# wenbowen123/iros20-6d-pose-tracking

Measured on AMD Instinct MI355X. Metric: RGB-D pair inferences/sec (176x176), higher is better.
Workload: dtype f32; 1 GPU; configs[1]: batch=64 synthetic 176x176 RGB-D pairs per GPU, random-init Se3TrackNet (reference state_dict surface), stage=full; pairs_per_gpu=64, global_batch=64, stage=full, frames=resident in HBM

## Files before the change

iros20-6d-pose-tracking_amd/csrc/api.cpp:

```cpp
#include <cmath>
#include <thread>
#include <type_traits>
#include <cstdio>
#include <cstdlib>
#include <chrono>
#include <cstring>
#include <map>
#include <mutex>
#include <set>
#include <string>
#include <vector>

#include "hip_buffers.h"
#include "pose_align_plan.h"
#include "pose_errors_plan.h"
#include "pose_grid_plan.h"
#include "pose_search_plan.h"
#include "se3tn_internal.h"
#include "tex_pyramid.h"
#include "track_plan.h"
#include "weights.h"

using namespace se3tn;

// ... 35 lines not shown
  const float* blob = nullptr;
  BlobLayout L;
  DeviceBuf<float> inA, inB;
  DeviceBuf<float> stem;
  DeviceBuf<float> pool, t64, q64;
  DeviceBuf<float> ab, ab_t;
  DeviceBuf<float> head, head_t;
  DeviceBuf<float> head_f;
  unsigned written = 0;
  InferPlan plan;
  DeviceBuf<float> logits;
  DeviceBuf<float> fcpart;
  bool keep_intermediates = false;
  int auto_tile_override[2] = {0, 0};
  int gemmp = -1;
  bool wino_fuse = true;
  DeviceBuf<float> part;
  int tail_parts_ch = 16;
  bool tail_parts = true;
  bool small_kernels = true;
  int wino_min_batch = SE3TN_WINOGRAD_DEFAULT_MIN_BATCH;
  int wino_tile = SE3TN_WINOGRAD_DEFAULT_TILE;
  int wino_tile_derived = 0;
  DeviceBuf<float> wino_u[4];
  DeviceBuf<float> wino_u6[4];
  const float* wino6_blob = nullptr;
  DeviceBuf<float> wino_v, wino_m;
  const float* wino_blob = nullptr;
  int wino64_min_batch = SE3TN_TRUNK_WINOGRAD_DEFAULT_MIN_BATCH;
  int wino64_min_fill = SE3TN_TRUNK_WINOGRAD_DEFAULT_MIN_FILL;
// ... 129 lines not shown
                                 c->wino64_u[i].get() + g * per_g, s.cin, s.cout, 2, st));
  }
  HIPCHK(hipStreamSynchronize(st));
  c->wino64_blob = c->blob;
  return SE3TN_OK;
}

static int wino_prepare(se3tn_ctx* c, hipStream_t st) {
  DeviceGuard dg(c->device);
  HIPCHK(dg.err);
  if (int rc = wino64_prepare(c, st)) return rc;
  if (c->wino_min_batch <= 0 || c->max_batch < c->wino_min_batch) return SE3TN_OK;
  if (!c->wino_v) {
    HIPCHK(c->wino_v.alloc(wino_ws_floats(c->max_batch)));
    HIPCHK(c->wino_m.alloc(wino_ws_floats(c->max_batch)));
    for (int i = 0; i < 4; ++i) {
      const Conv3& s = conv_specs()[kWinoConvs[i]];
      HIPCHK(c->wino_u[i].alloc((size_t)s.groups * 36 * s.cin * s.cout));
    }
  }
  const int tile = c->wino_tile == 2 ? 2 : 4;
  if (c->blob && (c->wino_tile == 6 || c->wino_tile == SE3TN_WINOGRAD_TILE_AUTO || c->wino_tile == SE3TN_WINOGRAD_TILE_6_4) &&
      c->wino6_blob != c->blob) {
    for (int i = 0; i < 4; ++i) {
      const Conv3& s = conv_specs()[kWinoConvs[i]];
      if (!c->wino_u6[i]) HIPCHK(c->wino_u6[i].alloc((size_t)s.groups * 64 * s.cin * s.cout));
      for (int g = 0; g < s.groups; ++g)
        HIPCHK(launch_wino_weights(c->blob + c->L.conv_w[kWinoConvs[i]] + (size_t)g * conv3_words(s.cin, s.cout),
                                   c->wino_u6[i].get() + (size_t)g * 64 * s.cin * s.cout, s.cin, s.cout, 6, st));
    }
// ... 145 lines not shown
const char* se3tn_last_error(void) { return g_err.c_str(); }

int se3tn_create(int device, int max_batch, se3tn_ctx** out) {
  if (!out || max_batch < 1) return fail(SE3TN_E_ARG, "se3tn_create: bad argument");
  if (max_batch > SE3TN_MAX_BATCH_LIMIT)
    return fail(SE3TN_E_ARG, "se3tn_create: max_batch " + std::to_string(max_batch) + " exceeds SE3TN_MAX_BATCH_LIMIT (" +
                                 std::to_string(SE3TN_MAX_BATCH_LIMIT) + "): run larger sets as several calls");
  se3tn_ctx* c = new se3tn_ctx();
  c->device = device;
  c->max_batch = max_batch;
  c->L = blob_layout();
  c->SL = split_layout();
  if (const char* e = std::getenv("SE3TN_WINOGRAD_AUTO_TILE_AB2")) c->auto_tile_override[0] = (std::atoi(e) == 4 || std::atoi(e) == 6) ? std::atoi(e) : 0;
  if (const char* e = std::getenv("SE3TN_WINOGRAD_AUTO_TILE_HEADS")) c->auto_tile_override[1] = (std::atoi(e) == 4 || std::atoi(e) == 6) ? std::atoi(e) : 0;
  if (const char* e = std::getenv("SE3TN_WINO_GEMMP")) c->gemmp = std::atoi(e) != 0 ? 1 : 0;
  if (const char* e = std::getenv("SE3TN_WINOGRAD_FUSE")) c->wino_fuse = std::atoi(e) != 0;
  if (const char* e = std::getenv("SE3TN_TRUNK_WINOGRAD")) c->wino64_min_batch = std::atoi(e);
  if (const char* e = std::getenv("SE3TN_TRUNK_WINOGRAD_FILL")) c->wino64_min_fill = std::atoi(e);
  for (int i = 0; i < 8; ++i) { c->mean[i] = 0.0; c->stdv[i] = 1.0; }
  if (device >= 0) {
    hipDeviceProp_t prop;
    hipError_t e = hipGetDeviceProperties(&prop, device);
    if (e != hipSuccess) { delete c; return hipfail(e, "hipGetDeviceProperties"); }
    if (std::strncmp(prop.gcnArchName, "gfx950", 6) != 0) {
      std::string a = prop.gcnArchName;
      delete c;
      return fail(SE3TN_E_DEVICE, "device is " + a + ", this library is built for gfx950 only");
    }
    if (prop.multiProcessorCount > 0) c->num_cus = prop.multiProcessorCount;
    e = hipSetDevice(device);
// ... 311 lines not shown
    a.per_img = 1;
    std::memcpy(a.img_off, ip->off, sizeof(a.img_off));
  }
}
static void fill_wino_args(se3tn_ctx* c, const ConvRow& r, int tile, int n, const float* W, bool split, WinoArgs& w) {
  const Conv3& s = conv_specs()[r.id];
  const int ws = wino_slot(r.id);
  w = WinoArgs{};
  w.in = tensor_ptr(c, r.in, split); w.bias = W + c->L.conv_b[r.id]; w.res = tensor_ptr(c, r.res, split); w.out = tensor_ptr(c, r.out, split);
  w.U = tile == 6 ? c->wino_u6[ws].get() : c->wino_u[ws].get();
  w.V = c->wino_v.get(); w.Mw = c->wino_m.get();
  w.in_ld = r.in.ld; w.res_ld = r.res.ld; w.out_ld = r.out.ld;
  w.m = tile; w.nf = (tile + 2) * (tile + 2);
  w.H = r.hin; w.W = r.hin; w.th = (r.hin + tile - 1) / tile; w.tw = w.th;
  w.n = n; w.T = n * w.th * w.tw;
  w.C = s.cin; w.Cout = s.cout; w.groups = s.groups;
  w.in_gs = r.in.gs; w.res_gs = r.res.gs; w.out_gs = r.out.gs; w.bias_gs = s.cout;
  w.u_gs = (long long)w.nf * s.cin * s.cout;
  if (split) {
    w.split = 1;
    w.U = c->wino_us[ws].get(); w.uscale = c->wino_usc[ws].get();
    w.overflow = c->overflow.get();
  }
}

static int infer_launch(se3tn_ctx* c, const float* A, const float* B, int n, int layout, float* trans, float* rot,
                        const double* poseA, double* poseB, void* stream);

int se3tn_enable_graphs(se3tn_ctx* c, int on) {
  if (!c || c->device < 0) return fail(SE3TN_E_ARG, "se3tn_enable_graphs: no device context");
// ... 1593 lines not shown
```

iros20-6d-pose-tracking_amd/csrc/se3tn_internal.h:

```cpp
#pragma once
#include <hip/hip_runtime.h>
#include <stddef.h>
#include <stdint.h>

#include "../../include/se3tracknet.h"
#include "infer_plan.h"

namespace se3tn {

struct BlobLayout {
  size_t stem_w;
  size_t stem_b;
  size_t conv_w[NUM_CONV3];
  size_t conv_b[NUM_CONV3];
  size_t fc_w;
  size_t fc_b;
  size_t total;
};

constexpr int HEADER_WORDS = 64;
constexpr uint32_t BLOB_MAGIC = 0x53453354u;
constexpr uint32_t BLOB_VERSION = 7;

struct SplitLayout {
// ... 85 lines not shown
  const float* res;
  float* out;
  float* V;
  float* Mw;
  int in_ld, res_ld, out_ld;
  int H, W;
  int m, nf;
  int th, tw;
  int n, T;
  int C, Cout, groups;
  int in_gs, res_gs, out_gs, bias_gs;
  long long u_gs;
  int split;
  const float* uscale;
  int* overflow;
};

struct TailArgs {
  const float* fc_w;
  const float* fc_b;
  float* logits;
  float* fcpart;
  float* trans;
  float* rot;
  const double* poseA;
  double* poseB;
  double tn, rn;
};

struct CropArgs {
// ... 230 lines not shown
```

iros20-6d-pose-tracking_amd/csrc/wino_mfma.hip:

```cpp
#include "mfma_common.h"
#include "pose_device.h"

#ifndef WINO4_VEC
#define WINO4_VEC 2
#endif
#ifndef WINO_MID_CS_AB
#define WINO_MID_CS_AB 32
#endif
#ifndef WINO_MID_CS_H
#define WINO_MID_CS_H 32
#endif

#ifdef SE3TN_GEMMP_TRACE
__device__ unsigned long long se3tn_gemmp_trace[8 * 64 * 5];
extern "C" int se3tn_debug_gemmp_trace(void* host_out, size_t bytes) {
  return (int)hipMemcpyFromSymbol(host_out, HIP_SYMBOL(se3tn_gemmp_trace), bytes, 0, hipMemcpyDeviceToHost);
}
#define GP_STAMP(K, I) if (blockIdx.x == 0 && lane == 0 && (K) < 64) ::se3tn_gemmp_trace[(wid * 64 + (K)) * 5 + (I)] = __builtin_amdgcn_s_memtime();
#else
#define GP_STAMP(K, I)
#endif
#ifdef SE3TN_WG_TRACE
__device__ unsigned long long se3tn_wg_trace[8 * 4096];
extern "C" int se3tn_debug_wg_trace(void* host_out, size_t bytes, int clear) {
// ... 87 lines not shown
  *reinterpret_cast<hv*>(p_ + 64) = l;
  return bad;
}

struct TileId { int t, cv, n, ty, tx; };
__device__ __forceinline__ TileId tile_of(int idx, int cvn, int th, int tw) {
  TileId r;
  r.cv = idx % cvn; r.t = idx / cvn;
  const int tpi = th * tw;
  r.n = r.t / tpi;
  const int rem = r.t - r.n * tpi;
  r.ty = rem / tw; r.tx = rem - r.ty * tw;
  return r;
}

template <int M, int VEC, int SP = 0>
__global__ __launch_bounds__(256) void wino_input_kernel(const WinoArgs a) {
  constexpr int N = M + 2;
  typedef typename VecT<VEC>::type vec;
  const int cvn = a.C / VEC;
  const int idx = blockIdx.x * 256 + threadIdx.x;
  if (idx >= a.T * cvn) return;
  const int g = blockIdx.y;
  const TileId id = tile_of(idx, cvn, a.th, a.tw);
  const int Hp = a.H + 2, Wp = a.W + 2;
  const float* __restrict__ src = a.in + (size_t)g * a.in_gs + (SP ? 0 : id.cv * VEC);
  float bt[N][N][VEC];
  if constexpr (M == 6) {
    static_assert(SP == 0, "F(6x6) is a float32 path");
#pragma unroll
// ... 37 lines not shown
      __builtin_memcpy(d[r][s], &v, sizeof(v));
    }
#pragma unroll
  for (int i = 0; i < N; ++i)
#pragma unroll
    for (int s = 0; s < N; ++s)
#pragma unroll
      for (int e = 0; e < VEC; ++e) {
        float acc = 0.f;
        bool first = true;
#pragma unroll
        for (int r = 0; r < N; ++r) axpy(acc, wino_bt<M>(i, r), d[r][s][e], first);
        bt[i][s][e] = acc;
      }
  }
  float* __restrict__ dst = a.V + ((size_t)g * a.nf * a.T + id.t) * a.C + (SP ? 0 : id.cv * VEC);
  const size_t fs = (size_t)a.T * a.C;
  bool bad = false;
#pragma unroll
  for (int i = 0; i < N; ++i)
#pragma unroll
    for (int j = 0; j < N; ++j) {
      float o[VEC];
#pragma unroll
      for (int e = 0; e < VEC; ++e) {
        float acc = 0.f;
        bool first = true;
#pragma unroll
        for (int s = 0; s < N; ++s) axpy(acc, wino_bt<M>(j, s), bt[i][s][e], first);
        o[e] = acc;
      }
      if (SP) {
        bad |= store_split_vec<VEC>(dst + (size_t)(N * i + j) * fs, 0, a.C, id.cv * VEC, o);
        continue;
      }
      vec v;
      __builtin_memcpy(&v, o, sizeof(v));
      *reinterpret_cast<vec*>(dst + (size_t)(N * i + j) * fs) = v;
    }
  if (SP && bad) atomicOr(a.overflow, 1);
}

template <int M, int VEC, int EPI, int SP = 0>
__global__ __launch_bounds__(256) void wino_output_kernel(const WinoArgs a) {
  constexpr int N = M + 2;
  typedef typename VecT<VEC>::type vec;
  const int cvn = a.Cout / VEC;
  const int idx = blockIdx.x * 256 + threadIdx.x;
  if (idx >= a.T * cvn) return;
  const int g = blockIdx.y;
  const TileId id = tile_of(idx, cvn, a.th, a.tw);
  const int Hp = a.H + 2, Wp = a.W + 2;
  const float* __restrict__ src = a.Mw + ((size_t)g * a.nf * a.T + id.t) * a.Cout + id.cv * VEC;
  const size_t fs = (size_t)a.T * a.Cout;
  float rr[M][M][VEC];
  if constexpr (EPI == 1 && SP == 0) {
    const float* __restrict__ res0 = a.res + (size_t)g * a.res_gs + id.cv * VEC;
#pragma unroll
    for (int i = 0; i < M; ++i)
#pragma unroll
      for (int j = 0; j < M; ++j) {
        int oy = M * id.ty + i, ox = M * id.tx + j;
        oy = oy < a.H ? oy : a.H - 1; ox = ox < a.W ? ox : a.W - 1;
        const vec v = *reinterpret_cast<const vec*>(res0 + (size_t)((id.n * Hp + oy + 1) * Wp + ox + 1) * a.res_ld);
        __builtin_memcpy(rr[i][j], &v, sizeof(v));
      }
  }
  float u[M][N][VEC];
#pragma unroll
  for (int s = 0; s < N; ++s) {
    float m[N][VEC];
#pragma unroll
    for (int r = 0; r < N; ++r) {
      const vec v = *reinterpret_cast<const vec*>(src + (size_t)(N * r + s) * fs);
      __builtin_memcpy(m[r], &v, sizeof(v));
    }
#pragma unroll
    for (int i = 0; i < M; ++i)
#pragma unroll
      for (int e = 0; e < VEC; ++e) {
        float acc = 0.f;
        bool first = true;
#pragma unroll
        for (int r = 0; r < N; ++r) axpy(acc, wino_at<M>(i, r), m[r][e], first);
        u[i][s][e] = acc;
      }
  }
  float b[VEC];
  {
    const vec v = *reinterpret_cast<const vec*>(a.bias + (size_t)g * a.bias_gs + id.cv * VEC);
    __builtin_memcpy(b, &v, sizeof(v));
  }
  const float* __restrict__ res = (EPI == 1) ? a.res + (size_t)g * a.res_gs + (SP ? 0 : id.cv * VEC) : nullptr;
  float* __restrict__ out = a.out + (size_t)g * a.out_gs + (SP ? 0 : id.cv * VEC);
  bool bad = false;
  if constexpr (SP == 0) __builtin_amdgcn_s_waitcnt(0x0F70);
#pragma unroll
  for (int i = 0; i < M; ++i)
#pragma unroll
    for (int j = 0; j < M; ++j) {
      const int oy = M * id.ty + i, ox = M * id.tx + j;
      if (oy >= a.H || ox >= a.W) continue;
      const size_t pix = (size_t)((id.n * Hp + oy + 1) * Wp + ox + 1);
      float r[VEC];
      if (EPI == 1) {
        if (SP) {
// ... 55 lines not shown
__global__ __launch_bounds__(256, 2) void wino_gemm_kernel(const WinoArgs a) {
  constexpr int BM = WM * PT * 32, BN = WN * CT * 32;
  constexpr int NCH = CIN / 32;
  constexpr int BUF = (BM + BN) * 32;
  static_assert(WM * WN == 4, "4 waves");
  extern __shared__ __attribute__((aligned(16))) float smem[];

  const int tid = threadIdx.x;
  const int lane = tid & 63;
  const int wid = __builtin_amdgcn_readfirstlane(tid >> 6);
  const int wm = wid / WN, wn = wid % WN;
  const int l31 = lane & 31, hh = lane >> 5;

  const int panels = a.Cout / BN, mtiles = (a.T + BM - 1) / BM;
  const int nt = blockIdx.x % panels, rest = blockIdx.x / panels;
  const int mt = rest % mtiles, b = rest / mtiles;
  const int g = b / a.nf, f = b - g * a.nf;
  const int m0 = mt * BM, n0 = nt * BN;
  const float* __restrict__ Vb = a.V + (size_t)b * a.T * CIN;
  const float* __restrict__ Ub = a.U + (size_t)g * a.u_gs + ((size_t)f * a.Cout + n0) * 32;
  const int mlast = a.T - 1;

  const int r0 = tid >> 3;
  const int c4 = (tid & 7) ^ ((r0 >> 1) & 7);
  unsigned pvoff[BM / 32];
#pragma unroll
  for (int j = 0; j < BM / 32; ++j) pvoff[j] = (unsigned)((min(m0 + r0 + 32 * j, mlast) * CIN + c4 * 4) * 4);
  const unsigned wvoff = (unsigned)((r0 * 32 + c4 * 4) * 4);
  const unsigned lds0 = __builtin_amdgcn_readfirstlane(lds_addr_of(smem));

#define ISSUE_TILE(CH, BUFI)                                                                         \
  {                                                                                                  \
    const float* pb_ = Vb + (CH) * 32;                                                               \
    const unsigned lb_ = lds0 + (unsigned)(((BUFI) * BUF + wid * 256) * 4);                          \
    _Pragma("unroll") for (int j_ = 0; j_ < BM / 32; ++j_) glds16<0>(pb_, pvoff[j_], lb_ + j_ * 4096); \
    const float* tb_ = Ub + (size_t)(CH) * a.nf * a.Cout * 32;                                       \
// ... 84 lines not shown
__global__ __launch_bounds__(512, 2) void wino_gemmp_kernel(const WinoArgs a, int total_tiles) {
  constexpr int BM = 128, BN = 256;
  constexpr int WN = 4, PT = 2, CT = 2;
  constexpr int VP = BM / 64;
  constexpr int NCH = CIN / 32;
  constexpr int BUF = (BM + BN) * 32;
  static_assert(NCH % 2 == 0, "the double buffer's parity must be the same at every tile start");
  extern __shared__ __attribute__((aligned(16))) float smem[];

  const int tid = threadIdx.x;
  const int lane = tid & 63;
  const int wid = __builtin_amdgcn_readfirstlane(tid >> 6);
  const int wm = wid / WN, wn = wid % WN;
  const int l31 = lane & 31, hh = lane >> 5;
  const int panels = a.Cout / BN, mtiles = (a.T + BM - 1) / BM, tpp = panels * mtiles;
  const int mlast = a.T - 1;

  const int r0 = tid >> 3;
  const int c4 = (tid & 7) ^ ((r0 >> 1) & 7);
  const unsigned wvoff = (unsigned)((r0 * 32 + c4 * 4) * 4);
  const unsigned lds0 = __builtin_amdgcn_readfirstlane(lds_addr_of(smem));

  auto decode = [&](int v, int& b, int& m0, int& n0) {
    const int xcd = v & 7, s = v >> 3;
    const int q = s / tpp, r = s - q * tpp;
    b = q * 8 + xcd;
    n0 = (r % panels) * BN;
    m0 = (r / panels) * BM;
  };
  const float* Vb;
  const float* Ub;
  unsigned pvoff[VP];
  auto set_tile = [&](int b, int m0, int n0) {
    const int g = b / a.nf, f = b - g * a.nf;
    Vb = a.V + (size_t)b * a.T * CIN;
    Ub = a.U + (size_t)g * a.u_gs + ((size_t)f * a.Cout + n0) * 32;
#pragma unroll
    for (int j = 0; j < VP; ++j) pvoff[j] = (unsigned)((min(m0 + r0 + 64 * j, mlast) * CIN + c4 * 4) * 4);
  };
#define ISSUE_TILEP(CH, BUFI)                                                                        \
  {                                                                                                  \
    const float* pb_ = Vb + (CH) * 32;                                                               \
    const unsigned lb_ = lds0 + (unsigned)(((BUFI) * BUF + wid * 256) * 4);                          \
    _Pragma("unroll") for (int j_ = 0; j_ < VP; ++j_) glds16<0>(pb_, pvoff[j_], lb_ + j_ * 8192);     \
    const float* tb_ = Ub + (size_t)(CH) * a.nf * a.Cout * 32;                                       \
    _Pragma("unroll") for (int j_ = 0; j_ < 4; ++j_) glds16<0>(tb_ + 2048 * j_, wvoff, lb_ + BM * 128 + j_ * 8192); \
  }

  const int X = (l31 >> 1) & 7;
  const int lo = (hh ^ (X & 1)) * 4, xk = X >> 1;
  const int fo0 = ((0 ^ xk) << 3) + lo, fo1 = ((1 ^ xk) << 3) + lo, fo2 = ((2 ^ xk) << 3) + lo, fo3 = ((3 ^ xk) << 3) + lo;

  f32x16 acc[PT][CT];
#pragma unroll
  for (int i = 0; i < PT; ++i)
#pragma unroll
    for (int j = 0; j < CT; ++j)
#pragma unroll
      for (int e = 0; e < 16; ++e) acc[i][j][e] = 0.f;

  int v = blockIdx.x;
  if (v >= total_tiles) return;
  int b, m0, n0;
  decode(v, b, m0, n0);
  set_tile(b, m0, n0);
  ISSUE_TILEP(0, 0)
  wait_dma_and_barrier();

  int kstep_ = 0;
  (void)kstep_;
  while (true) {
    const int vn = v + gridDim.x;
    const bool more = vn < total_tiles;
    const int cb = b, cm0 = m0, cn0 = n0;
#pragma unroll 1
    for (int ch = 0; ch < NCH; ++ch) {
      const int buf = ch & 1;
      GP_STAMP(kstep_, 0)
      if (ch + 1 < NCH) {
        ISSUE_TILEP(ch + 1, buf ^ 1)
      } else if (more) {
        decode(vn, b, m0, n0);
        set_tile(b, m0, n0);
        ISSUE_TILEP(0, buf ^ 1)
      }
      GP_STAMP(kstep_, 1)
      const float* pP = smem + buf * BUF + (wm * PT * 32 + l31) * 32;
      const float* pW = smem + buf * BUF + (BM + wn * CT * 32 + l31) * 32;
#define FOG(G) ((G) == 0 ? fo0 : (G) == 1 ? fo1 : (G) == 2 ? fo2 : fo3)
#define PXF(G) *reinterpret_cast<const float4*>(pP + i * 1024 + FOG(G))
#define WTF(G) *reinterpret_cast<const float4*>(pW + j * 1024 + FOG(G))
      SE3TN_MMA_GROUP(PT, CT, PXF(0), WTF(0))
      SE3TN_MMA_GROUP(PT, CT, PXF(1), WTF(1))
      SE3TN_MMA_GROUP(PT, CT, PXF(2), WTF(2))
      SE3TN_MMA_GROUP(PT, CT, PXF(3), WTF(3))
#undef PXF
#undef WTF
#undef FOG
// ... 3 lines not shown
        GP_STAMP(kstep_, 3)
        __syncthreads();
      }
      GP_STAMP(kstep_, 4)
      ++kstep_;
    }
    float* __restrict__ Mb = a.Mw + (size_t)cb * a.T * a.Cout;
#pragma unroll
    for (int i = 0; i < PT; ++i) {
      const int m = cm0 + (wm * PT + i) * 32 + l31;
#pragma unroll
      for (int j = 0; j < CT; ++j)
#pragma unroll
        for (int q = 0; q < 4; ++q) {
          const int c = cn0 + (wn * CT + j) * 32 + q * 8 + hh * 4;
          if (m <= mlast)
            *reinterpret_cast<float4*>(Mb + (size_t)m * a.Cout + c) =
                make_float4(acc[i][j][4 * q + 0], acc[i][j][4 * q + 1], acc[i][j][4 * q + 2], acc[i][j][4 * q + 3]);
#pragma unroll
          for (int e = 0; e < 4; ++e) acc[i][j][4 * q + e] = 0.f;
        }
    }
    if (!more) break;
    v = vn;
  }
#undef ISSUE_TILEP
}

template <> struct VecT<1> { typedef float type; };

template <int M, int TH, int CS, int VEC, int SP = 0>
__global__ __launch_bounds__(((TH * TH * (CS / VEC) + 63) / 64) * 64) void wino_mid_kernel(const WinoArgs a, float* __restrict__ keep) {
  constexpr int N = M + 2, HP = M * TH + 2, NT = TH * TH, CP = CS / VEC, ITEMS = NT * CP;
  typedef typename VecT<VEC>::type vec;
  static_assert(SP == 0 || (M == 4 && VEC == 2), "the f16x3 blocks are F(4x4) with channel pairs");
  extern __shared__ __attribute__((aligned(16))) float act[];
  const int n = blockIdx.x, c0 = blockIdx.y * CS, g = blockIdx.z;
  const int tid = threadIdx.x;
  for (int i = tid; i < HP * HP * CS / 4; i += blockDim.x) reinterpret_cast<float4*>(act)[i] = make_float4(0.f, 0.f, 0.f, 0.f);
  __syncthreads();
  const int tile = tid / CP, cp = tid - tile * CP;
  const int ty = tile / TH, tx = tile - ty * TH;
  const bool active = tid < ITEMS;
  const int t = n * NT + tile;
  const int Hp = a.H + 2, Wp = a.W + 2;
  if (active) {
    const float* __restrict__ src = a.Mw + ((size_t)g * a.nf * a.T + t) * a.Cout + c0 + cp * VEC;
    const size_t fs = (size_t)a.T * a.Cout;
    float u[M][N][VEC];
#pragma unroll
    for (int s = 0; s < N; ++s) {
      float m[N][VEC];
#pragma unroll
      for (int r = 0; r < N; ++r) {
        const vec v = *reinterpret_cast<const vec*>(src + (size_t)(N * r + s) * fs);
        __builtin_memcpy(m[r], &v, sizeof(v));
      }
#pragma unroll
      for (int i = 0; i < M; ++i)
#pragma unroll
        for (int e = 0; e < VEC; ++e) {
          float acc = 0.f;
          bool first = true;
#pragma unroll
          for (int r = 0; r < N; ++r) axpy(acc, wino_at<M>(i, r), m[r][e], first);
          u[i][s][e] = acc;
        }
    }
    float b[VEC];
    {
      const vec v = *reinterpret_cast<const vec*>(a.bias + (size_t)g * a.bias_gs + c0 + cp * VEC);
      __builtin_memcpy(b, &v, sizeof(v));
    }
    float* __restrict__ kp = keep ? keep + (size_t)g * a.out_gs + c0 + cp * VEC : nullptr;
#pragma unroll
    for (int i = 0; i < M; ++i)
#pragma unroll
      for (int j = 0; j < M; ++j) {
        const int oy = M * ty + i, ox = M * tx + j;
        if (oy >= a.H || ox >= a.W) continue;
        float o[VEC];
#pragma unroll
        for (int e = 0; e < VEC; ++e) {
          float acc = 0.f;
          bool first = true;
#pragma unroll
          for (int s = 0; s < N; ++s) axpy(acc, wino_at<M>(j, s), u[i][s][e], first);
          acc += b[e];
// ... 15 lines not shown
      for (int r = 0; r < N; ++r) {
        const vec v = *reinterpret_cast<const vec*>(act + ((M * ty + r) * HP + M * tx + s) * CS + cp * VEC);
        __builtin_memcpy(d[r], &v, sizeof(v));
      }
#pragma unroll
      for (int i = 0; i < N; ++i)
#pragma unroll
        for (int e = 0; e < VEC; ++e) {
          float acc = 0.f;
          bool first = true;
#pragma unroll
          for (int r = 0; r < N; ++r) axpy(acc, wino_bt<M>(i, r), d[r][e], first);
          bt[i][s][e] = acc;
        }
    }
    float* __restrict__ dst = a.V + ((size_t)g * a.nf * a.T + t) * a.C + (SP ? 0 : c0 + cp * VEC);
    const size_t fs = (size_t)a.T * a.C;
    bool bad = false;
#pragma unroll
    for (int i = 0; i < N; ++i)
#pragma unroll
      for (int j = 0; j < N; ++j) {
        float o[VEC];
#pragma unroll
        for (int e = 0; e < VEC; ++e) {
          float acc = 0.f;
          bool first = true;
#pragma unroll
          for (int s = 0; s < N; ++s) axpy(acc, wino_bt<M>(j, s), bt[i][s][e], first);
          o[e] = acc;
        }
        if constexpr (SP != 0) {
          bad |= store_split_vec<VEC>(dst + (size_t)(N * i + j) * fs, 0, a.C, c0 + cp * VEC, o);
        } else {
          vec v;
          __builtin_memcpy(&v, o, sizeof(v));
          *reinterpret_cast<vec*>(dst + (size_t)(N * i + j) * fs) = v;
        }
      }
    if (SP && bad) atomicOr(a.overflow, 1);
  }
}

__device__ __forceinline__ float wave_sum64(float v) {
#pragma unroll
  for (int o = 32; o > 0; o >>= 1) v += __shfl_xor(v, o, 64);
  return v;
}

template <int M, int TH, int CS, int SP = 0>
__global__ __launch_bounds__(((TH * TH * (CS / 2) + 63) / 64) * 64) void wino_tail_kernel(const WinoArgs a, float* __restrict__ keep,
                                                                                         const float* __restrict__ fc_w,
                                                                                         float* __restrict__ fcpart) {
  constexpr int N = M + 2, NT = TH * TH, CP = CS / 2, ITEMS = NT * CP;
  static_assert(SP == 0 || M == 4, "the f16x3 blocks are F(4x4)");
  static_assert(CP == 32, "the FC partials are reduced inside one half-wave");
  __shared__ float red[NT][CP][2];
  const int n = blockIdx.x, sl = blockIdx.y, g = blockIdx.z, tid = threadIdx.x;
  const int tile = tid / CP, cp = tid - tile * CP;
  const int c = sl * CS + cp * 2;
  const int Hp = a.H + 2, Wp = a.W + 2;
  if (tid < ITEMS) {
    const int ty = tile / TH, tx = tile - ty * TH;
    const size_t fs = (size_t)a.T * a.Cout;
    const float* __restrict__ src = a.Mw + ((size_t)g * a.nf * a.T + n * NT + tile) * a.Cout + c;
    const float* __restrict__ res = a.res + (size_t)g * a.res_gs + (SP ? 0 : c);
    float* __restrict__ kp = keep ? keep + (size_t)g * a.out_gs + c : nullptr;
    const float2 b = *reinterpret_cast<const float2*>(a.bias + (size_t)g * a.bias_gs + c);
    float2 rr[M][M];
    if constexpr (SP == 0) {
#pragma unroll
      for (int i = 0; i < M; ++i)
#pragma unroll
        for (int j = 0; j < M; ++j) {
          int oy = M * ty + i, ox = M * tx + j;
          oy = oy < a.H ? oy : a.H - 1; ox = ox < a.W ? ox : a.W - 1;
          rr[i][j] = *reinterpret_cast<const float2*>(res + (size_t)((n * Hp + oy + 1) * Wp + ox + 1) * a.res_ld);
        }
    }
    float u[M][N][2];
#pragma unroll
    for (int s = 0; s < N; ++s) {
      float m[N][2];
#pragma unroll
      for (int r = 0; r < N; ++r) {
        const float2 v = *reinterpret_cast<const float2*>(src + (size_t)(N * r + s) * fs);
        m[r][0] = v.x; m[r][1] = v.y;
      }
#pragma unroll
      for (int i = 0; i < M; ++i)
#pragma unroll
        for (int e = 0; e < 2; ++e) {
          float acc = 0.f;
          bool first = true;
#pragma unroll
          for (int r = 0; r < N; ++r) axpy(acc, wino_at<M>(i, r), m[r][e], first);
          u[i][s][e] = acc;
        }
    }
    float sum[2] = {0.f, 0.f};
#pragma unroll
    for (int i = 0; i < M; ++i)
#pragma unroll
      for (int j = 0; j < M; ++j) {
        const int oy = M * ty + i, ox = M * tx + j;
        if (oy >= a.H || ox >= a.W) continue;
        const size_t pix = (size_t)((n * Hp + oy + 1) * Wp + ox + 1);
        float2 r;
        if (SP) {
          float rr[2];
          load_split_vec<2>(res, pix, a.res_ld, c, rr);
          r = make_float2(rr[0], rr[1]);
        } else {
// ... 70 lines not shown
}

template <int CIN, int WM, int WN, int PT, int CT, int MM = MM_F32>
static hipError_t launch_gemm(const WinoArgs& a, hipStream_t st) {
  static PerDeviceOnce attr;
  auto kern = wino_gemm_kernel<CIN, WM, WN, PT, CT, MM>;
  constexpr int BM = WM * PT * 32, BN = WN * CT * 32;
  const size_t lds = 2 * (BM + BN) * 32 * sizeof(float);
  bool* done = attr.current();
  if (!done || !*done) {
    hipError_t e = hipFuncSetAttribute(reinterpret_cast<const void*>(kern),
                                       hipFuncAttributeMaxDynamicSharedMemorySize, (int)lds);
    if (e != hipSuccess) return e;
    if (done) *done = true;
  }
  const int grid = (a.Cout / BN) * ((a.T + BM - 1) / BM) * a.groups * a.nf;
  hipLaunchKernelGGL(kern, dim3(grid), dim3(256), lds, st, a);
  return hipGetLastError();
}

template <int CIN>
static hipError_t launch_gemmp(const WinoArgs& a, int total_tiles, int grid, hipStream_t st) {
  static PerDeviceOnce attr;
  auto kern = wino_gemmp_kernel<CIN>;
  const size_t lds = 2 * (128 + 256) * 32 * sizeof(float);
  bool* done = attr.current();
  if (!done || !*done) {
    hipError_t e = hipFuncSetAttribute(reinterpret_cast<const void*>(kern), hipFuncAttributeMaxDynamicSharedMemorySize, (int)lds);
    if (e != hipSuccess) return e;
    if (done) *done = true;
  }
  hipLaunchKernelGGL(kern, dim3(grid), dim3(512), lds, st, a, total_tiles);
  return hipGetLastError();
}

template <int CIN>
static hipError_t launch_gemm_planned(const WinoArgs& a, const GemmPlan& g, hipStream_t st) {
  if (g.kind == GemmPlan::PERSISTENT) {
    if (a.split || a.Cout % 256 != 0 || g.grid < 1 || g.tiles != (a.Cout / 256) * ((a.T + 127) / 128) * a.groups * a.nf) return hipErrorInvalidValue;
    return launch_gemmp<CIN>(a, g.tiles, g.grid, st);
  }
  if (g.kind != GemmPlan::ROWS96 && g.kind != GemmPlan::ROWS128) return hipErrorInvalidValue;
  const bool r96 = g.kind == GemmPlan::ROWS96;
  if (a.split) return r96 ? launch_gemm<CIN, 1, 4, 3, 1, MM_F16X3>(a, st) : launch_gemm<CIN, 2, 2, 2, 2, MM_F16X3>(a, st);
  return r96 ? launch_gemm<CIN, 1, 4, 3, 1>(a, st) : launch_gemm<CIN, 2, 2, 2, 2>(a, st);
}

template <int M, int VEC>
static hipError_t launch_transformed(const WinoArgs& a, const GemmPlan& g, int epi, hipStream_t st) {
  hipLaunchKernelGGL((wino_input_kernel<M, VEC>), dim3((a.T * (a.C / VEC) + 255) / 256, a.groups), dim3(256), 0, st, a);
  hipError_t e = hipGetLastError();
  if (e != hipSuccess) return e;
  e = a.C == 256 ? launch_gemm_planned<256>(a, g, st) : launch_gemm_planned<512>(a, g, st);
  if (e != hipSuccess) return e;
// ... 93 lines not shown
```

Baseline: 41850 pairs/s.

## Skip dead Winograd F(6,3) transform planes for partial boundary tiles

For 6x6-output Winograd tiles, the last row and column of the 8x8 transform only contribute to outputs that are needed when the tile fits fully inside the image. The change reorders V/M rows per plane class (finite, row-infinity, column-infinity), so tiles that do not need those planes are packed out of the GEMM range. The input transform, GEMM (standard and persistent), and output transform then skip the unneeded rows. This is meant to reduce GEMM work and memory traffic on the boundary planes, at the cost of more complex indexing and tile decoding. A debug poison option is also added.

```diff
diff --git a/iros20-6d-pose-tracking_amd/csrc/api.cpp b/iros20-6d-pose-tracking_amd/csrc/api.cpp
--- a/iros20-6d-pose-tracking_amd/csrc/api.cpp
+++ b/iros20-6d-pose-tracking_amd/csrc/api.cpp
@@ -73,6 +73,8 @@
   bool keep_intermediates = false;
   int auto_tile_override[2] = {0, 0};
   int gemmp = -1;
+  bool wino_full_planes = false;
+  bool wino_poison = false;
   bool wino_fuse = true;
   DeviceBuf<float> part;
   int tail_parts_ch = 16;
@@ -232,6 +234,10 @@
   if (!c->wino_v) {
     HIPCHK(c->wino_v.alloc(wino_ws_floats(c->max_batch)));
     HIPCHK(c->wino_m.alloc(wino_ws_floats(c->max_batch)));
+    if (c->wino_poison) {
+      HIPCHK(hipMemset(c->wino_v.get(), 0xFF, c->wino_v.count() * sizeof(float)));
+      HIPCHK(hipMemset(c->wino_m.get(), 0xFF, c->wino_m.count() * sizeof(float)));
+    }
     for (int i = 0; i < 4; ++i) {
       const Conv3& s = conv_specs()[kWinoConvs[i]];
       HIPCHK(c->wino_u[i].alloc((size_t)s.groups * 36 * s.cin * s.cout));
@@ -407,6 +413,8 @@
   if (const char* e = std::getenv("SE3TN_WINOGRAD_AUTO_TILE_AB2")) c->auto_tile_override[0] = (std::atoi(e) == 4 || std::atoi(e) == 6) ? std::atoi(e) : 0;
   if (const char* e = std::getenv("SE3TN_WINOGRAD_AUTO_TILE_HEADS")) c->auto_tile_override[1] = (std::atoi(e) == 4 || std::atoi(e) == 6) ? std::atoi(e) : 0;
   if (const char* e = std::getenv("SE3TN_WINO_GEMMP")) c->gemmp = std::atoi(e) != 0 ? 1 : 0;
+  if (const char* e = std::getenv("SE3TN_WINO_FULL_PLANES")) c->wino_full_planes = std::atoi(e) != 0;
+  if (const char* e = std::getenv("SE3TN_WINO_POISON")) c->wino_poison = std::atoi(e) != 0;
   if (const char* e = std::getenv("SE3TN_WINOGRAD_FUSE")) c->wino_fuse = std::atoi(e) != 0;
   if (const char* e = std::getenv("SE3TN_TRUNK_WINOGRAD")) c->wino64_min_batch = std::atoi(e);
   if (const char* e = std::getenv("SE3TN_TRUNK_WINOGRAD_FILL")) c->wino64_min_fill = std::atoi(e);
@@ -748,6 +756,7 @@
   w.m = tile; w.nf = (tile + 2) * (tile + 2);
   w.H = r.hin; w.W = r.hin; w.th = (r.hin + tile - 1) / tile; w.tw = w.th;
   w.n = n; w.T = n * w.th * w.tw;
+  w.trim = plan_wino_trim(w.H, w.W, tile, w.th, w.tw, n, c->wino_full_planes);
   w.C = s.cin; w.Cout = s.cout; w.groups = s.groups;
   w.in_gs = r.in.gs; w.res_gs = r.res.gs; w.out_gs = r.out.gs; w.bias_gs = s.cout;
   w.u_gs = (long long)w.nf * s.cin * s.cout;
diff --git a/iros20-6d-pose-tracking_amd/csrc/se3tn_internal.h b/iros20-6d-pose-tracking_amd/csrc/se3tn_internal.h
--- a/iros20-6d-pose-tracking_amd/csrc/se3tn_internal.h
+++ b/iros20-6d-pose-tracking_amd/csrc/se3tn_internal.h
@@ -5,6 +5,7 @@
 
 #include "../../include/se3tracknet.h"
 #include "infer_plan.h"
+#include "wino_trim_plan.h"
 
 namespace se3tn {
 
@@ -123,6 +124,7 @@
   int split;
   const float* uscale;
   int* overflow;
+  WinoTrim trim;
 };
 
 struct TailArgs {
diff --git a/iros20-6d-pose-tracking_amd/csrc/wino_mfma.hip b/iros20-6d-pose-tracking_amd/csrc/wino_mfma.hip
--- a/iros20-6d-pose-tracking_amd/csrc/wino_mfma.hip
+++ b/iros20-6d-pose-tracking_amd/csrc/wino_mfma.hip
@@ -125,6 +125,92 @@
   return r;
 }
 
+struct TileRows { int ra, rc; bool need_r, need_c; };
+template <int M>
+__device__ __forceinline__ TileRows tile_rows(const WinoArgs& a, int t, int img, int ty, int tx) {
+  TileRows r{t, t, true, true};
+  if constexpr (M == 6) {
+    r.ra = wino_trim_row(a.trim, WINO_PLANES_FINITE, a.n, a.th, a.tw, img, ty, tx);
+    r.rc = wino_trim_row(a.trim, WINO_PLANES_COL_INF, a.n, a.th, a.tw, img, ty, tx);
+    r.need_r = ty < a.trim.ny;
+    r.need_c = tx < a.trim.nx;
+  }
+  return r;
+}
+
+template <int VEC>
+__device__ __forceinline__ void out_rows6(const float* __restrict__ src_a, const float* __restrict__ src_c, size_t fs, const TileRows& tr,
+                                          float (&u)[6][8][VEC]) {
+  typedef typename VecT<VEC>::type vec;
+  float mr[8][VEC], mc[7][VEC];
+  if (tr.need_r) {
+#pragma unroll
+    for (int s = 0; s < 8; ++s) {
+      const vec v = *reinterpret_cast<const vec*>(src_a + (size_t)(56 + s) * fs);
+      __builtin_memcpy(mr[s], &v, sizeof(v));
+    }
+  }
+  if (tr.need_c) {
+#pragma unroll
+    for (int r = 0; r < 7; ++r) {
+      const vec v = *reinterpret_cast<const vec*>(src_c + (size_t)(8 * r + 7) * fs);
+      __builtin_memcpy(mc[r], &v, sizeof(v));
+    }
+  }
+  float m[7][7][VEC];
+  const float* __restrict__ p = src_a;
+#pragma unroll
+  for (int r = 0; r < 7; ++r) {
+#pragma unroll
+    for (int s = 0; s < 7; ++s) {
+      const vec v = *reinterpret_cast<const vec*>(p);
+      __builtin_memcpy(m[r][s], &v, sizeof(v));
+      p += fs;
+    }
+    p += fs;
+  }
+  __builtin_amdgcn_sched_barrier(0);
+#pragma unroll
+  for (int s = 0; s < 7; ++s)
+#pragma unroll
+    for (int i = 0; i < 6; ++i)
+#pragma unroll
+      for (int e = 0; e < VEC; ++e) {
+        float acc = 0.f;
+        bool first = true;
+#pragma unroll
+        for (int r = 0; r < 7; ++r) axpy(acc, wino_at<6>(i, r), m[r][s][e], first);
+        u[i][s][e] = acc;
+      }
+#pragma unroll
+  for (int i = 0; i < 6; ++i)
+#pragma unroll
+    for (int e = 0; e < VEC; ++e) u[i][7][e] = 0.f;
+  if (tr.need_c) {
+#pragma unroll
+    for (int i = 0; i < 6; ++i)
+#pragma unroll
+      for (int e = 0; e < VEC; ++e) {
+        float acc = 0.f;
+        bool first = true;
+#pragma unroll
+        for (int r = 0; r < 7; ++r) axpy(acc, wino_at<6>(i, r), mc[r][e], first);
+        u[i][7][e] = acc;
+      }
+  }
+  if (tr.need_r) {
+#pragma unroll
+    for (int s = 0; s < 8; ++s)
+#pragma unroll
+      for (int i = 0; i < 6; ++i)
+#pragma unroll
+        for (int e = 0; e < VEC; ++e) {
+          bool first = false;
+          axpy(u[i][s][e], wino_at<6>(i, 7), mr[s][e], first);
+        }
+  }
+}
+
 template <int M, int VEC, int SP = 0>
 __global__ __launch_bounds__(256) void wino_input_kernel(const WinoArgs a) {
   constexpr int N = M + 2;
@@ -192,13 +278,18 @@
         bt[i][s][e] = acc;
       }
   }
-  float* __restrict__ dst = a.V + ((size_t)g * a.nf * a.T + id.t) * a.C + (SP ? 0 : id.cv * VEC);
+  const TileRows tr = tile_rows<M>(a, id.t, id.n, id.ty, id.tx);
+  float* __restrict__ dst = a.V + ((size_t)g * a.nf * a.T + tr.ra) * a.C + (SP ? 0 : id.cv * VEC);
+  float* __restrict__ dst_c = a.V + ((size_t)g * a.nf * a.T + tr.rc) * a.C + (SP ? 0 : id.cv * VEC);
   const size_t fs = (size_t)a.T * a.C;
   bool bad = false;
 #pragma unroll
   for (int i = 0; i < N; ++i)
 #pragma unroll
     for (int j = 0; j < N; ++j) {
+      if constexpr (M == 6) {
+        if (i == N - 1 ? !tr.need_r : (j == N - 1 && !tr.need_c)) continue;
+      }
       float o[VEC];
 #pragma unroll
       for (int e = 0; e < VEC; ++e) {
@@ -208,13 +299,14 @@
         for (int s = 0; s < N; ++s) axpy(acc, wino_bt<M>(j, s), bt[i][s][e], first);
         o[e] = acc;
       }
+      float* __restrict__ d = (M == 6 && j == N - 1 && i < N - 1 ? dst_c : dst) + (size_t)(N * i + j) * fs;
       if (SP) {
-        bad |= store_split_vec<VEC>(dst + (size_t)(N * i + j) * fs, 0, a.C, id.cv * VEC, o);
+        bad |= store_split_vec<VEC>(d, 0, a.C, id.cv * VEC, o);
         continue;
       }
       vec v;
       __builtin_memcpy(&v, o, sizeof(v));
-      *reinterpret_cast<vec*>(dst + (size_t)(N * i + j) * fs) = v;
+      *reinterpret_cast<vec*>(d) = v;
     }
   if (SP && bad) atomicOr(a.overflow, 1);
 }
@@ -229,7 +321,8 @@
   const int g = blockIdx.y;
   const TileId id = tile_of(idx, cvn, a.th, a.tw);
   const int Hp = a.H + 2, Wp = a.W + 2;
-  const float* __restrict__ src = a.Mw + ((size_t)g * a.nf * a.T + id.t) * a.Cout + id.cv * VEC;
+  const TileRows tr = tile_rows<M>(a, id.t, id.n, id.ty, id.tx);
+  const float* __restrict__ src = a.Mw + ((size_t)g * a.nf * a.T + tr.ra) * a.Cout + id.cv * VEC;
   const size_t fs = (size_t)a.T * a.Cout;
   float rr[M][M][VEC];
   if constexpr (EPI == 1 && SP == 0) {
@@ -244,30 +337,34 @@
         __builtin_memcpy(rr[i][j], &v, sizeof(v));
       }
   }
-  float u[M][N][VEC];
-#pragma unroll
-  for (int s = 0; s < N; ++s) {
-    float m[N][VEC];
-#pragma unroll
-    for (int r = 0; r < N; ++r) {
-      const vec v = *reinterpret_cast<const vec*>(src + (size_t)(N * r + s) * fs);
-      __builtin_memcpy(m[r], &v, sizeof(v));
-    }
-#pragma unroll
-    for (int i = 0; i < M; ++i)
-#pragma unroll
-      for (int e = 0; e < VEC; ++e) {
-        float acc = 0.f;
-        bool first = true;
-#pragma unroll
-        for (int r = 0; r < N; ++r) axpy(acc, wino_at<M>(i, r), m[r][e], first);
-        u[i][s][e] = acc;
-      }
-  }
   float b[VEC];
   {
     const vec v = *reinterpret_cast<const vec*>(a.bias + (size_t)g * a.bias_gs + id.cv * VEC);
     __builtin_memcpy(b, &v, sizeof(v));
+  }
+  float u[M][N][VEC];
+  if constexpr (M == 6) {
+    out_rows6<VEC>(src, a.Mw + ((size_t)g * a.nf * a.T + tr.rc) * a.Cout + id.cv * VEC, fs, tr, u);
+  } else {
+#pragma unroll
+  for (int s = 0; s < N; ++s) {
+    float m[N][VEC];
+#pragma unroll
+    for (int r = 0; r < N; ++r) {
+      const vec v = *reinterpret_cast<const vec*>(src + (size_t)(N * r + s) * fs);
+      __builtin_memcpy(m[r], &v, sizeof(v));
+    }
+#pragma unroll
+    for (int i = 0; i < M; ++i)
+#pragma unroll
+      for (int e = 0; e < VEC; ++e) {
+        float acc = 0.f;
+        bool first = true;
+#pragma unroll
+        for (int r = 0; r < N; ++r) axpy(acc, wino_at<M>(i, r), m[r][e], first);
+        u[i][s][e] = acc;
+      }
+  }
   }
   const float* __restrict__ res = (EPI == 1) ? a.res + (size_t)g * a.res_gs + (SP ? 0 : id.cv * VEC) : nullptr;
   float* __restrict__ out = a.out + (size_t)g * a.out_gs + (SP ? 0 : id.cv * VEC);
@@ -353,12 +450,29 @@
 
   const int panels = a.Cout / BN, mtiles = (a.T + BM - 1) / BM;
   const int nt = blockIdx.x % panels, rest = blockIdx.x / panels;
-  const int mt = rest % mtiles, b = rest / mtiles;
+  int mt = rest % mtiles, b = rest / mtiles, mlast = a.T - 1;
+  if (a.trim.on) {
+    const int tf = mtiles, tr = wino_row_tiles(a.trim, WINO_PLANES_ROW_INF, BM), tc = wino_row_tiles(a.trim, WINO_PLANES_COL_INF, BM);
+    const int rowsz = 7 * tf + tc, per_g = 7 * rowsz + 8 * tr;
+    const int gq = rest / per_g, rem = rest - gq * per_g;
+    if (gq >= a.groups) return;
+    int r, s, cls;
+    if (rem < 7 * rowsz) {
+      r = rem / rowsz;
+      const int x = rem - r * rowsz;
+      if (x < 7 * tf) { s = x / tf; mt = x - s * tf; cls = WINO_PLANES_FINITE; }
+      else { s = 7; mt = x - 7 * tf; cls = WINO_PLANES_COL_INF; }
+    } else {
+      const int x = rem - 7 * rowsz;
+      r = 7; s = x / tr; mt = x - s * tr; cls = WINO_PLANES_ROW_INF;
+    }
+    b = gq * 64 + 8 * r + s;
+    mlast = a.trim.live[cls] - 1;
+  }
   const int g = b / a.nf, f = b - g * a.nf;
   const int m0 = mt * BM, n0 = nt * BN;
   const float* __restrict__ Vb = a.V + (size_t)b * a.T * CIN;
   const float* __restrict__ Ub = a.U + (size_t)g * a.u_gs + ((size_t)f * a.Cout + n0) * 32;
-  const int mlast = a.T - 1;
 
   const int r0 = tid >> 3;
   const int c4 = (tid & 7) ^ ((r0 >> 1) & 7);
@@ -473,16 +587,30 @@
   const int wm = wid / WN, wn = wid % WN;
   const int l31 = lane & 31, hh = lane >> 5;
   const int panels = a.Cout / BN, mtiles = (a.T + BM - 1) / BM, tpp = panels * mtiles;
-  const int mlast = a.T - 1;
+  const int xcd = blockIdx.x & 7;
+  const int cls_a = xcd == 7 ? WINO_PLANES_COL_INF : WINO_PLANES_FINITE;
+  const int tpa = panels * wino_row_tiles(a.trim, cls_a, BM), tpb = panels * wino_row_tiles(a.trim, WINO_PLANES_ROW_INF, BM);
+  const int spg = 7 * tpa + tpb;
+  const int slots = a.trim.on ? a.groups * spg : (total_tiles - xcd + 7) >> 3;
 
   const int r0 = tid >> 3;
   const int c4 = (tid & 7) ^ ((r0 >> 1) & 7);
   const unsigned wvoff = (unsigned)((r0 * 32 + c4 * 4) * 4);
   const unsigned lds0 = __builtin_amdgcn_readfirstlane(lds_addr_of(smem));
 
-  auto decode = [&](int v, int& b, int& m0, int& n0) {
-    const int xcd = v & 7, s = v >> 3;
-    const int q = s / tpp, r = s - q * tpp;
+  auto decode = [&](int v, int& b, int& m0, int& n0, int& mlast) {
+    const int s = v >> 3;
+    int q, r;
+    mlast = a.T - 1;
+    if (a.trim.on) {
+      const int gq = s / spg, rem = s - gq * spg;
+      int pr;
+      if (rem < 7 * tpa) { pr = rem / tpa; r = rem - pr * tpa; mlast = a.trim.live[cls_a] - 1; }
+      else { pr = 7; r = rem - 7 * tpa; mlast = a.trim.live[WINO_PLANES_ROW_INF] - 1; }
+      q = gq * 8 + pr;
+    } else {
+      q = s / tpp; r = s - q * tpp;
+    }
     b = q * 8 + xcd;
     n0 = (r % panels) * BN;
     m0 = (r / panels) * BM;
@@ -490,7 +618,7 @@
   const float* Vb;
   const float* Ub;
   unsigned pvoff[VP];
-  auto set_tile = [&](int b, int m0, int n0) {
+  auto set_tile = [&](int b, int m0, int n0, int mlast) {
     const int g = b / a.nf, f = b - g * a.nf;
     Vb = a.V + (size_t)b * a.T * CIN;
     Ub = a.U + (size_t)g * a.u_gs + ((size_t)f * a.Cout + n0) * 32;
@@ -519,10 +647,10 @@
       for (int e = 0; e < 16; ++e) acc[i][j][e] = 0.f;
 
   int v = blockIdx.x;
-  if (v >= total_tiles) return;
-  int b, m0, n0;
-  decode(v, b, m0, n0);
-  set_tile(b, m0, n0);
+  if ((v >> 3) >= slots) return;
+  int b, m0, n0, mlast;
+  decode(v, b, m0, n0, mlast);
+  set_tile(b, m0, n0, mlast);
   ISSUE_TILEP(0, 0)
   wait_dma_and_barrier();
 
@@ -530,8 +658,8 @@
   (void)kstep_;
   while (true) {
     const int vn = v + gridDim.x;
-    const bool more = vn < total_tiles;
-    const int cb = b, cm0 = m0, cn0 = n0;
+    const bool more = (vn >> 3) < slots;
+    const int cb = b, cm0 = m0, cn0 = n0, cmlast = mlast;
 #pragma unroll 1
     for (int ch = 0; ch < NCH; ++ch) {
       const int buf = ch & 1;
@@ -539,8 +667,8 @@
       if (ch + 1 < NCH) {
         ISSUE_TILEP(ch + 1, buf ^ 1)
       } else if (more) {
-        decode(vn, b, m0, n0);
-        set_tile(b, m0, n0);
+        decode(vn, b, m0, n0, mlast);
+        set_tile(b, m0, n0, mlast);
         ISSUE_TILEP(0, buf ^ 1)
       }
       GP_STAMP(kstep_, 1)
@@ -574,7 +702,7 @@
 #pragma unroll
         for (int q = 0; q < 4; ++q) {
           const int c = cn0 + (wn * CT + j) * 32 + q * 8 + hh * 4;
-          if (m <= mlast)
+          if (m <= cmlast)
             *reinterpret_cast<float4*>(Mb + (size_t)m * a.Cout + c) =
                 make_float4(acc[i][j][4 * q + 0], acc[i][j][4 * q + 1], acc[i][j][4 * q + 2], acc[i][j][4 * q + 3]);
 #pragma unroll
@@ -604,34 +732,39 @@
   const bool active = tid < ITEMS;
   const int t = n * NT + tile;
   const int Hp = a.H + 2, Wp = a.W + 2;
+  const TileRows tr = tile_rows<M>(a, t, n, ty, tx);
   if (active) {
-    const float* __restrict__ src = a.Mw + ((size_t)g * a.nf * a.T + t) * a.Cout + c0 + cp * VEC;
+    const float* __restrict__ src = a.Mw + ((size_t)g * a.nf * a.T + tr.ra) * a.Cout + c0 + cp * VEC;
     const size_t fs = (size_t)a.T * a.Cout;
-    float u[M][N][VEC];
-#pragma unroll
-    for (int s = 0; s < N; ++s) {
-      float m[N][VEC];
-#pragma unroll
-      for (int r = 0; r < N; ++r) {
-        const vec v = *reinterpret_cast<const vec*>(src + (size_t)(N * r + s) * fs);
-        __builtin_memcpy(m[r], &v, sizeof(v));
-      }
-#pragma unroll
-      for (int i = 0; i < M; ++i)
-#pragma unroll
-        for (int e = 0; e < VEC; ++e) {
-          float acc = 0.f;
-          bool first = true;
-#pragma unroll
-          for (int r = 0; r < N; ++r) axpy(acc, wino_at<M>(i, r), m[r][e], first);
-          u[i][s][e] = acc;
-        }
-    }
     float b[VEC];
     {
       const vec v = *reinterpret_cast<const vec*>(a.bias + (size_t)g * a.bias_gs + c0 + cp * VEC);
       __builtin_memcpy(b, &v, sizeof(v));
     }
+    float u[M][N][VEC];
+    if constexpr (M == 6) {
+      out_rows6<VEC>(src, a.Mw + ((size_t)g * a.nf * a.T + tr.rc) * a.Cout + c0 + cp * VEC, fs, tr, u);
+    } else {
+#pragma unroll
+    for (int s = 0; s < N; ++s) {
+      float m[N][VEC];
+#pragma unroll
+      for (int r = 0; r < N; ++r) {
+        const vec v = *reinterpret_cast<const vec*>(src + (size_t)(N * r + s) * fs);
+        __builtin_memcpy(m[r], &v, sizeof(v));
+      }
+#pragma unroll
+      for (int i = 0; i < M; ++i)
+#pragma unroll
+        for (int e = 0; e < VEC; ++e) {
+          float acc = 0.f;
+          bool first = true;
+#pragma unroll
+          for (int r = 0; r < N; ++r) axpy(acc, wino_at<M>(i, r), m[r][e], first);
+          u[i][s][e] = acc;
+        }
+    }
+    }
     float* __restrict__ kp = keep ? keep + (size_t)g * a.out_gs + c0 + cp * VEC : nullptr;
 #pragma unroll
     for (int i = 0; i < M; ++i)
@@ -677,13 +810,18 @@
           bt[i][s][e] = acc;
         }
     }
-    float* __restrict__ dst = a.V + ((size_t)g * a.nf * a.T + t) * a.C + (SP ? 0 : c0 + cp * VEC);
+    float* __restrict__ dst = a.V + ((size_t)g * a.nf * a.T + tr.ra) * a.C + (SP ? 0 : c0 + cp * VEC);
+    float* __restrict__ dst_c = a.V + ((size_t)g * a.nf * a.T + tr.rc) * a.C + (SP ? 0 : c0 + cp * VEC);
     const size_t fs = (size_t)a.T * a.C;
     bool bad = false;
 #pragma unroll
     for (int i = 0; i < N; ++i)
 #pragma unroll
       for (int j = 0; j < N; ++j) {
+        if constexpr (M == 6) {
+          if (i == N - 1 ? !tr.need_r : (j == N - 1 && !tr.need_c)) continue;
+        }
+        float* __restrict__ d = (M == 6 && j == N - 1 && i < N - 1 ? dst_c : dst) + (size_t)(N * i + j) * fs;
         float o[VEC];
 #pragma unroll
         for (int e = 0; e < VEC; ++e) {
@@ -694,11 +832,11 @@
           o[e] = acc;
         }
         if constexpr (SP != 0) {
-          bad |= store_split_vec<VEC>(dst + (size_t)(N * i + j) * fs, 0, a.C, c0 + cp * VEC, o);
+          bad |= store_split_vec<VEC>(d, 0, a.C, c0 + cp * VEC, o);
         } else {
           vec v;
           __builtin_memcpy(&v, o, sizeof(v));
-          *reinterpret_cast<vec*>(dst + (size_t)(N * i + j) * fs) = v;
+          *reinterpret_cast<vec*>(d) = v;
         }
       }
     if (SP && bad) atomicOr(a.overflow, 1);
@@ -726,7 +864,8 @@
   if (tid < ITEMS) {
     const int ty = tile / TH, tx = tile - ty * TH;
     const size_t fs = (size_t)a.T * a.Cout;
-    const float* __restrict__ src = a.Mw + ((size_t)g * a.nf * a.T + n * NT + tile) * a.Cout + c;
+    const TileRows tr = tile_rows<M>(a, n * NT + tile, n, ty, tx);
+    const float* __restrict__ src = a.Mw + ((size_t)g * a.nf * a.T + tr.ra) * a.Cout + c;
     const float* __restrict__ res = a.res + (size_t)g * a.res_gs + (SP ? 0 : c);
     float* __restrict__ kp = keep ? keep + (size_t)g * a.out_gs + c : nullptr;
     const float2 b = *reinterpret_cast<const float2*>(a.bias + (size_t)g * a.bias_gs + c);
@@ -742,6 +881,9 @@
         }
     }
     float u[M][N][2];
+    if constexpr (M == 6) {
+      out_rows6<2>(src, a.Mw + ((size_t)g * a.nf * a.T + tr.rc) * a.Cout + c, fs, tr, u);
+    } else {
 #pragma unroll
     for (int s = 0; s < N; ++s) {
       float m[N][2];
@@ -760,6 +902,7 @@
           for (int r = 0; r < N; ++r) axpy(acc, wino_at<M>(i, r), m[r][e], first);
           u[i][s][e] = acc;
         }
+    }
     }
     float sum[2] = {0.f, 0.f};
 #pragma unroll
@@ -860,7 +1003,8 @@
     if (e != hipSuccess) return e;
     if (done) *done = true;
   }
-  const int grid = (a.Cout / BN) * ((a.T + BM - 1) / BM) * a.groups * a.nf;
+  if (a.trim.on && a.nf != 64) return hipErrorInvalidValue;
+  const int grid = a.trim.on ? wino_live_tiles(a.trim, a.Cout, a.groups, BM, BN) : (a.Cout / BN) * ((a.T + BM - 1) / BM) * a.groups * a.nf;
   hipLaunchKernelGGL(kern, dim3(grid), dim3(256), lds, st, a);
   return hipGetLastError();
 }
@@ -884,6 +1028,7 @@
 static hipError_t launch_gemm_planned(const WinoArgs& a, const GemmPlan& g, hipStream_t st) {
   if (g.kind == GemmPlan::PERSISTENT) {
     if (a.split || a.Cout % 256 != 0 || g.grid < 1 || g.tiles != (a.Cout / 256) * ((a.T + 127) / 128) * a.groups * a.nf) return hipErrorInvalidValue;
+    if (a.trim.on && (a.nf != 64 || g.grid % 8 != 0)) return hipErrorInvalidValue;
     return launch_gemmp<CIN>(a, g.tiles, g.grid, st);
   }
   if (g.kind != GemmPlan::ROWS96 && g.kind != GemmPlan::ROWS128) return hipErrorInvalidValue;
diff --git a/iros20-6d-pose-tracking_amd/csrc/wino_trim_plan.h b/iros20-6d-pose-tracking_amd/csrc/wino_trim_plan.h
--- /dev/null
+++ b/iros20-6d-pose-tracking_amd/csrc/wino_trim_plan.h
@@ -0,0 +1,52 @@
+#pragma once
+
+#if defined(__HIPCC__) || defined(__CUDACC__)
+#define SE3TN_TRIM_FN __host__ __device__ __forceinline__
+#else
+#define SE3TN_TRIM_FN inline
+#endif
+
+namespace se3tn {
+
+enum WinoPlaneClass { WINO_PLANES_FINITE = 0, WINO_PLANES_ROW_INF = 1, WINO_PLANES_COL_INF = 2 };
+
+struct WinoTrim {
+  int on;
+  int ny, nx;
+  int live[3];
+};
+
+SE3TN_TRIM_FN int wino_plane_class(int f) { return (f >> 3) == 7 ? WINO_PLANES_ROW_INF : (f & 7) == 7 ? WINO_PLANES_COL_INF : WINO_PLANES_FINITE; }
+
+SE3TN_TRIM_FN int wino_trim_row(const WinoTrim& t, int cls, int n, int th, int tw, int img, int ty, int tx) {
+  if (!t.on) return (img * th + ty) * tw + tx;
+  return cls == WINO_PLANES_COL_INF ? (tx * th + ty) * n + img : (ty * tw + tx) * n + img;
+}
+
+SE3TN_TRIM_FN bool wino_tile_needs(const WinoTrim& t, int f, int ty, int tx) {
+  const int cls = wino_plane_class(f);
+  return cls == WINO_PLANES_ROW_INF ? ty < t.ny : cls == WINO_PLANES_COL_INF ? tx < t.nx : true;
+}
+
+inline WinoTrim plan_wino_trim(int H, int W, int m, int th, int tw, int n, bool full) {
+  WinoTrim t;
+  const int T = n * th * tw;
+  t.on = 0; t.ny = th; t.nx = tw;
+  t.live[0] = t.live[1] = t.live[2] = T;
+  if (m != 6 || full) return t;
+  t.on = 1; t.ny = 0; t.nx = 0;
+  for (int ty = 0; ty < th; ++ty) t.ny += (m * ty + m - 1 < H) ? 1 : 0;
+  for (int tx = 0; tx < tw; ++tx) t.nx += (m * tx + m - 1 < W) ? 1 : 0;
+  t.live[WINO_PLANES_ROW_INF] = t.ny * tw * n;
+  t.live[WINO_PLANES_COL_INF] = t.nx * th * n;
+  return t;
+}
+
+SE3TN_TRIM_FN int wino_row_tiles(const WinoTrim& t, int cls, int bm) { return (t.live[cls] + bm - 1) / bm; }
+
+inline int wino_live_tiles(const WinoTrim& t, int cout, int groups, int bm, int bn) {
+  return (cout / bn) * groups *
+         (49 * wino_row_tiles(t, WINO_PLANES_FINITE, bm) + 8 * wino_row_tiles(t, WINO_PLANES_ROW_INF, bm) + 7 * wino_row_tiles(t, WINO_PLANES_COL_INF, bm));
+}
+
+}
```

After: 42060 pairs/s, median of 6. No clear change (+0.5%).
